# nnanhuang/S3Gaussian

Measured on AMD Instinct MI355X. Metric: train_iters_per_sec, higher is better.
Workload: dtype f32

## Files before the change

### include/s3g_mlp.h

```cpp
#ifndef S3G_MLP_H
#define S3G_MLP_H
#include <stddef.h>
#ifdef __cplusplus
extern "C" {
#endif

typedef struct s3g_mlp_params {
  float *W0, *b0;
  float *P1, *pb1;
  float *P2, *pb2;
  float *S1, *sb1;
  float *S2, *sb2;
  float *D0, *db0;
  float *D1, *db1;
  float *D2, *db2;
} s3g_mlp_params;

size_t s3g_deform_mlp_stash_bytes(int P);
size_t s3g_deform_mlp_pack_bytes(void);

int s3g_deform_mlp_forward(const s3g_mlp_params* w, int P, const float* features, float* dx, float* dshs, float* feat,
                           float* stash, int save_activations, void* stream);

int s3g_deform_mlp_backward(const s3g_mlp_params* w, int P, const float* features, const float* stash, const float* g_dx,
                            const float* g_dshs, const float* g_feat, float* g_features, const s3g_mlp_params* gw,
                            float* workspace, void* stream);

size_t s3g_deform_mlp_wgrad_partial_bytes(void);
int s3g_deform_mlp_backward_ordered(const s3g_mlp_params* w, int P, const float* features, const float* stash, const float* g_dx,
                                    const float* g_dshs, const float* g_feat, float* g_features, const s3g_mlp_params* gw,
                                    float* workspace, float* wgrad_partials, void* stream);

enum { S3G_MLP_F32 = 0, S3G_MLP_BF16X3 = 1, S3G_MLP_BF16X3_ONTHEFLY = 2 };
int s3g_deform_mlp_set_arithmetic(int mode);
int s3g_deform_mlp_get_arithmetic(void);

#include "s3g_hexplane.h"
size_t s3g_deform_infer_workspace_bytes(const s3g_hexplane_desc* d);
int s3g_deform_infer(const s3g_hexplane_desc* d, const s3g_mlp_params* w, int P, const float* xyz, const float* time,
                     const unsigned int* proc_order, float* dx, float* dshs, void* workspace, void* stream);
int s3g_deform_infer_split(const s3g_hexplane_desc* d, const s3g_mlp_params* w, int P, const float* xyz, const float* time,
                           const unsigned int* proc_order, float* dx, float* dshs, void* workspace, void* stream);

#ifdef __cplusplus
}
#endif
#endif
```

### s3gaussian_amd/_lib.py

```python
from __future__ import annotations

import ctypes as C
import os
import subprocess

_HERE = os.path.dirname(os.path.abspath(__file__))
LIB_PATH = os.environ.get("S3G_LIB_PATH") or os.path.join(_HERE, "lib", "libs3g.so")
CSRC_DIR = os.path.join(_HERE, "csrc")

ABI_VERSION = 15

RESIZE_FN = C.CFUNCTYPE(C.c_void_p, C.c_void_p, C.c_size_t)


class RasterInputs(C.Structure):
    _fields_ = [
        ("P", C.c_int), ("D", C.c_int), ("M", C.c_int), ("width", C.c_int), ("height", C.c_int),
        ("background", C.c_void_p), ("means3D", C.c_void_p), ("shs", C.c_void_p), ("colors_precomp", C.c_void_p),
        ("opacities", C.c_void_p), ("scales", C.c_void_p), ("scale_modifier", C.c_float), ("rotations", C.c_void_p),
        ("cov3D_precomp", C.c_void_p), ("viewmatrix", C.c_void_p), ("projmatrix", C.c_void_p), ("cam_pos", C.c_void_p),
        ("tan_fovx", C.c_float), ("tan_fovy", C.c_float), ("prefiltered", C.c_int), ("debug", C.c_int),
    ]


class DensifyAccum(C.Structure):
# ... 106 lines not shown
    if _torch is None:
        _torch, _raw_stream, _cur_device = _bind_fast_paths()
    if _cur_device is not None and getattr(dev, "index", None) is not None and _cur_device() == dev.index:
        return _NULL
    return _torch.cuda.device(dev)


def check(code: int) -> None:
    if code != 0:
        msg = lib().s3g_last_error().decode("utf-8", "replace")
        if code == 1:
            raise Exception(msg)
        raise RuntimeError(f"libs3g error {code}: {msg}")


EXPORTED_SYMBOLS = ["s3g_raster_forward", "s3g_raster_forward_reuse", "s3g_raster_forward_decompose", "s3g_raster_forward2", "s3g_raster_forward_async", "s3g_raster_arena_bytes", "s3g_adam_step_guarded", "s3g_raster_backward", "s3g_raster_backward_workspace_bytes", "s3g_raster_backward2", "s3g_raster_backward2_workspace_bytes", "s3g_hexplane_forward_workspace_bytes", "s3g_knn_workspace_bytes", "s3g_knn_mean_dist2", "s3g_hexplane_forward", "s3g_hexplane_backward", "s3g_hexplane_backward_algo", "s3g_hexplane_backward_workspace_bytes", "s3g_hexplane_backward_scratch_rows", "s3g_hexplane_debug_walk_mask", "s3g_hexplane_set_deterministic", "s3g_hexplane_get_deterministic", "s3g_hexplane_sort_state_words", "s3g_profile_enable", "s3g_profile_read", "s3g_ssim_forward", "s3g_ssim_backward", "s3g_plane_regulation", "s3g_scale_unless_one", "s3g_pixel_losses_forward", "s3g_pixel_losses_combine", "s3g_pixel_losses_backward", "s3g_glue_forward", "s3g_glue_backward", "s3g_deform_mlp_forward", "s3g_deform_mlp_backward", "s3g_deform_mlp_backward_ordered", "s3g_deform_mlp_wgrad_partial_bytes", "s3g_deform_mlp_stash_bytes", "s3g_deform_mlp_pack_bytes", "s3g_deform_mlp_set_arithmetic", "s3g_deform_mlp_get_arithmetic", "s3g_deform_infer", "s3g_deform_infer_split", "s3g_deform_infer_workspace_bytes", "s3g_adam_step", "s3g_densify_stats", "s3g_densify_stats_guarded", "s3g_density_count_words", "s3g_density_classify_densify", "s3g_density_classify_prune", "s3g_density_scan", "s3g_density_apply", "s3g_density_reset_opacity", "s3g_image_metrics_workspace_bytes", "s3g_image_metrics", "s3g_scene_flow_workspace_bytes", "s3g_scene_flow_colors", "s3g_raster_backward_accum", "s3g_raster_backward2_accum", "s3g_mark_visible", "s3g_raster_set_exact_cull", "s3g_raster_get_exact_cull", "s3g_raster_set_bin_band", "s3g_raster_set_backward_wave_bounds", "s3g_last_error", "s3g_abi_version"]
```

### s3gaussian_amd/csrc/mlp.hip

```cpp
#include "mlp_dev.hpp"

namespace s3g {

__global__ void __launch_bounds__(256) mlp_pack_kernel(const s3g_mlp_params w, float* __restrict__ packed) {
  const int k = blockIdx.x, tid = threadIdx.x;
  float* dst = packed + (size_t)k * SLAB;
  if (k == NSLAB) {
    float* bl = packed + (size_t)NSLAB * SLAB;
    const float* src[8] = {w.b0, w.pb1, w.sb1, w.pb2, w.sb2, w.db0, w.db1, w.db2};
    const int n[8] = {64, 64, 64, 3, 48, 64, 64, 3};
    for (int e = tid; e < 8 * 64; e += 256) bl[e] = (e & 63) < n[e >> 6] ? src[e >> 6][e & 63] : 0.f;
    return;
  }
  const float* W = k <= 1 ? w.W0 : k == 2 ? w.P1 : k == 3 ? w.S1 : k == 4 ? w.P2 : k == 5 ? w.S2 : k == 6 ? w.D0 : k == 7 ? w.D1 : w.D2;
  const int out = (k == 4 || k == 8) ? 3 : (k == 5 ? 48 : 64), outpad = (k == 4 || k == 8) ? 32 : 64;
  const int in = k <= 1 ? FEAT : HID, in0 = k == 1 ? 64 : 0, ld = outpad + 1;
  for (int e = tid; e < SLAB; e += 256) dst[e] = 0.f;
  __syncthreads();
  for (int e = tid; e < outpad * 64; e += 256) {
    const int o = e / 64, i = e % 64;
    dst[i * ld + o] = o < out ? W[(size_t)o * in + in0 + i] : 0.f;
  }
}
void mlp_pack_launch(const s3g_mlp_params& w, float* packed, hipStream_t stream) {
// ... 96 lines not shown
      head3_fw(WSLAB(8), BIAS(7), acc, o3, ln);
      store3(o3, a.feat, p0, npts, ln);
    }
    }
    __builtin_amdgcn_sched_barrier(0);
    cur = nxt;
  }
}

struct MlpBwdArgs {
  int P;
  const float* packed;
  const uint32_t* maskbits;
  const float *g_dx, *g_dshs, *g_feat;
  float *g_x, *ws;
};

struct BwdIn {
  float gd[3], gf[3];
  float4 gs[6];
  uint32_t bits[5];
};

template <bool SPLIT>
__global__ void __launch_bounds__(NWAVE * 64) mlp_backward_kernel(const MlpBwdArgs a) {
  extern __shared__ __attribute__((aligned(16))) float lds[];
  const int lane = threadIdx.x & 63, wave = threadIdx.x >> 6;
  load_weights(lds, a.packed, wave, lane);
  const int ntiles = (a.P + MT - 1) / MT;
  const size_t PS = (size_t)a.P * HID;
// ... 20 lines not shown
  };
  const int stride = gridDim.x * NWAVE, t0 = blockIdx.x * NWAVE + wave;
  BwdIn cur, nxt;
  if (t0 < ntiles) issue(cur, t0);
  for (int tile = t0; tile < ntiles; tile += stride) {
    issue(nxt, min(tile + stride, ntiles - 1));
    __builtin_amdgcn_sched_barrier(0);
    const int p0 = tile * MT, npts = min(MT, a.P - p0);
    f32x16 ghid[2], g[2], acc[2], g3[1];
    acc_zero<2>(ghid);
    if (dino) {
      head3(g3, cur.gf);
      acc_zero<2>(acc);
      gemm_reg_t<2, 1, 3>(WSLAB(8), 33, g3, acc, lane);
      masked_bits<2, false>(g, acc, cur.bits[4]);
      act_store<HID, 2, false>(g, a.ws + 0 * PS, 0, p0, npts, lane);
      acc_zero<2>(acc);
      gemm_bw<SPLIT, 2, 2>(WSLAB(7), 65, g, acc, lane);
      masked_bits<2, false>(g, acc, cur.bits[3]);
      act_store<HID, 2, false>(g, a.ws + 1 * PS, 0, p0, npts, lane);
      gemm_bw<SPLIT, 2, 2>(WSLAB(6), 65, g, ghid, lane);
    }
    head3(g3, cur.gd);
    acc_zero<2>(acc);
    gemm_reg_t<2, 1, 3>(WSLAB(4), 33, g3, acc, lane);
    masked_bits<2, false>(g, acc, cur.bits[1]);
    act_store<HID, 2, false>(g, a.ws + 2 * PS, 0, p0, npts, lane);
    acc_zero<2>(acc);
    gemm_bw<SPLIT, 2, 2>(WSLAB(2), 65, g, acc, lane);
    {
      f32x16 gs[2], t[2];
#pragma unroll
      for (int c = 0; c < 8; c++) {
        const float4 v = c < 6 ? cur.gs[c < 6 ? c : 0] : make_float4(0.f, 0.f, 0.f, 0.f);
        gs[c >> 2][4 * (c & 3) + 0] = v.x; gs[c >> 2][4 * (c & 3) + 1] = v.y;
        gs[c >> 2][4 * (c & 3) + 2] = v.z; gs[c >> 2][4 * (c & 3) + 3] = v.w;
      }
      acc_zero<2>(t);
      gemm_bw<SPLIT, 2, 2>(WSLAB(5), 65, gs, t, lane);
      masked_bits<2, false>(g, t, cur.bits[2]);
    }
    act_store<HID, 2, false>(g, a.ws + 3 * PS, 0, p0, npts, lane);
// ... 156 lines not shown
  if (t0 < ntiles) issue(cur, t0);
  for (int tile = t0; tile < ntiles; tile += stride) {
    issue(nxt, min(tile + stride, ntiles - 1));
    __builtin_amdgcn_sched_barrier(0);
    const int p0 = tile * MT, npts = min(MT, a.P - p0);
    int ln = lane;
    asm volatile("" : "+v"(ln));
    f32x16 ghid[2], g[2], acc[2], g3[1];
    ActSplit<2> gsp;
    acc_zero<2>(ghid);
    if (dino) {
      head3(g3, cur.gf);
      acc_zero<2>(acc);
      gemm_reg_t<2, 1, 3>(lds + tbw::D2T, tbw::H3LD, g3, acc, ln);
      masked_bits<2, false>(g, acc, cur.bits[4]);
      act_store<HID, 2, false>(g, a.ws + 0 * PS, 0, p0, npts, ln);
      acc_zero<2>(acc);
      act_split<2, false>(gsp, g);
      gemm_split<2, 2>(wsplit + tbw::D1T, 4, 0, gsp, acc, ln);
      masked_bits<2, false>(g, acc, cur.bits[3]);
      act_store<HID, 2, false>(g, a.ws + 1 * PS, 0, p0, npts, ln);
      act_split<2, false>(gsp, g);
      gemm_split<2, 2>(wsplit + tbw::D0T, 4, 0, gsp, ghid, ln);
    }
    head3(g3, cur.gd);
    acc_zero<2>(acc);
    gemm_reg_t<2, 1, 3>(lds + tbw::P2T, tbw::H3LD, g3, acc, ln);
    masked_bits<2, false>(g, acc, cur.bits[1]);
    act_store<HID, 2, false>(g, a.ws + 2 * PS, 0, p0, npts, ln);
    acc_zero<2>(acc);
    act_split<2, false>(gsp, g);
#pragma unroll
    for (int ks = 0; ks < 4; ks++)
#pragma unroll
      for (int mbo = 0; mbo < 2; mbo++) {
        const float* wr = lds + tbw::P1T + (32 * mbo + (ln & 31)) * tbw::P1LD + 4 * (ln >> 5) + 16 * ks;
        const float4 lo = *reinterpret_cast<const float4*>(wr);
        const float4 hi = *reinterpret_cast<const float4*>(wr + 8);
        const float v[8] = {lo.x, lo.y, lo.z, lo.w, hi.x, hi.y, hi.z, hi.w};
        acc[mbo] = mfma_split(acc[mbo], split8(v), gsp.b[ks >> 1][ks & 1]);
      }
    {
      f32x16 gs[2], t[2];
#pragma unroll
// ... 164 lines not shown
extern "C" size_t s3g_deform_mlp_stash_bytes(int P) {
  return ((size_t)PACK_TOTAL + (size_t)5 * (size_t)(P > 0 ? P : 0) * HID + mask_words(P)) * sizeof(float);
}
extern "C" size_t s3g_deform_mlp_pack_bytes(void) { return (size_t)PACK_TOTAL * sizeof(float); }

static std::atomic<int> g_mlp_arithmetic{S3G_MLP_F32};
extern "C" int s3g_deform_mlp_set_arithmetic(int mode) {
  if (mode != S3G_MLP_F32 && mode != S3G_MLP_BF16X3 && mode != S3G_MLP_BF16X3_ONTHEFLY) {
    set_error("s3g_deform_mlp_set_arithmetic: mode must be S3G_MLP_F32, S3G_MLP_BF16X3 or S3G_MLP_BF16X3_ONTHEFLY");
    return S3G_ERR_INVALID_ARG;
  }
  g_mlp_arithmetic.store(mode, std::memory_order_relaxed);
  return S3G_OK;
}
extern "C" int s3g_deform_mlp_get_arithmetic(void) { return g_mlp_arithmetic.load(std::memory_order_relaxed); }

static int mlp_set_attrs() {
  static std::atomic<uint64_t> done{0};
  if (device_needs_setup(done)) {
    S3G_HIP_CHECK(hipFuncSetAttribute((const void*)mlp_forward_kernel<false>, hipFuncAttributeMaxDynamicSharedMemorySize, MLP_LDS_FLOATS * 4));
    S3G_HIP_CHECK(hipFuncSetAttribute((const void*)mlp_backward_kernel<false>, hipFuncAttributeMaxDynamicSharedMemorySize, MLP_LDS_FLOATS * 4));
    S3G_HIP_CHECK(hipFuncSetAttribute((const void*)mlp_forward_kernel<true>, hipFuncAttributeMaxDynamicSharedMemorySize, MLP_LDS_FLOATS * 4));
    S3G_HIP_CHECK(hipFuncSetAttribute((const void*)mlp_backward_kernel<true>, hipFuncAttributeMaxDynamicSharedMemorySize, MLP_LDS_FLOATS * 4));
    S3G_HIP_CHECK(hipFuncSetAttribute((const void*)mlp_forward_presplit_kernel, hipFuncAttributeMaxDynamicSharedMemorySize, tpw::WORDS * 4));
    S3G_HIP_CHECK(hipFuncSetAttribute((const void*)mlp_backward_presplit_kernel, hipFuncAttributeMaxDynamicSharedMemorySize, tbw::WORDS * 4));
    device_setup_done(done);
  }
  return S3G_OK;
}

// ... 33 lines not shown
}

static int mlp_backward_impl(const s3g_mlp_params* w, int P, const float* features, const float* stash_, const float* g_dx,
                             const float* g_dshs, const float* g_feat, float* g_features, const s3g_mlp_params* gw, float* workspace,
                             float* partials, void* stream_) {
  if (!w || !gw || P < 0 || (P > 0 && (!features || !stash_ || !g_dx || !g_dshs || !g_features || !workspace))) {
    set_error("s3g_deform_mlp_backward: bad argument");
    return S3G_ERR_INVALID_ARG;
  }
  if (P == 0) return S3G_OK;
  if (int e = mlp_set_attrs()) return e;
  hipStream_t stream = (hipStream_t)stream_;
  const float* stash = stash_ + PACK_TOTAL;
  MlpBwdArgs b;
  b.P = P; b.packed = stash_; b.maskbits = reinterpret_cast<const uint32_t*>(stash + (size_t)5 * P * HID); b.g_dx = g_dx; b.g_dshs = g_dshs; b.g_feat = g_feat; b.g_x = g_features; b.ws = workspace;
  const int ntiles = (P + MT - 1) / MT;
  const int blocks = min((ntiles + NWAVE - 1) / NWAVE, 256);
  const int arith = g_mlp_arithmetic.load(std::memory_order_relaxed);
  float* img = const_cast<float*>(stash_) + PACK_FLOATS + tpw::WORDS;
  if (arith == S3G_MLP_BF16X3)
    hipLaunchKernelGGL(mlp_pack_presplit_bwd_kernel, dim3((tbw::WORDS + 255) / 256), dim3(256), 0, stream, *w, reinterpret_cast<uint32_t*>(img));
  else
    mlp_pack_launch(*w, const_cast<float*>(stash_), stream);
  profile_begin(S3G_PROFILE_MLP_BACKWARD, stream);
  if (arith == S3G_MLP_BF16X3) {
    MlpBwdArgs sb = b;
    sb.packed = img;
    hipLaunchKernelGGL(mlp_backward_presplit_kernel, dim3(blocks), dim3(NWAVE * 64), tbw::WORDS * 4, stream, sb);
  } else if (arith != S3G_MLP_F32)
    hipLaunchKernelGGL(mlp_backward_kernel<true>, dim3(blocks), dim3(NWAVE * 64), MLP_LDS_FLOATS * 4, stream, b);
  else
    hipLaunchKernelGGL(mlp_backward_kernel<false>, dim3(blocks), dim3(NWAVE * 64), MLP_LDS_FLOATS * 4, stream, b);
  profile_end(S3G_PROFILE_MLP_BACKWARD, stream, (double)P, 0.0);
  S3G_HIP_CHECK(hipGetLastError());
  profile_begin(S3G_PROFILE_MLP_WGRAD, stream);
  if (int e = mlp_wgrad_launch(P, features, stash, workspace, g_dx, g_dshs, g_feat, gw, partials, stream)) return e;
  profile_end(S3G_PROFILE_MLP_WGRAD, stream, (double)P, 0.0);
  return S3G_OK;
}

extern "C" int s3g_deform_mlp_backward(const s3g_mlp_params* w, int P, const float* features, const float* stash_,
                                       const float* g_dx, const float* g_dshs, const float* g_feat, float* g_features,
                                       const s3g_mlp_params* gw, float* workspace, void* stream_) {
  return mlp_backward_impl(w, P, features, stash_, g_dx, g_dshs, g_feat, g_features, gw, workspace, nullptr, stream_);
}

extern "C" int s3g_deform_mlp_backward_ordered(const s3g_mlp_params* w, int P, const float* features, const float* stash_,
                                               const float* g_dx, const float* g_dshs, const float* g_feat, float* g_features,
                                               const s3g_mlp_params* gw, float* workspace, float* wgrad_partials, void* stream_) {
  if (!wgrad_partials && P > 0) {
    set_error("s3g_deform_mlp_backward_ordered: wgrad_partials is NULL");
// ... 5 lines not shown
```

### s3gaussian_amd/csrc/mlp_dev.hpp

```cpp
#pragma once
#include "common.hpp"

#include "../../include/s3g_mlp.h"

namespace s3g {

typedef float f32x16 __attribute__((ext_vector_type(16)));

constexpr int MT = 32;
constexpr int HID = 64;
constexpr int FEAT = 128;

__device__ __forceinline__ constexpr int rrow(int r) { return (r & 3) + 8 * (r >> 2); }
__device__ __forceinline__ int acc_row(int reg, int lane) { return rrow(reg) + 4 * (lane >> 5); }

template <int MBO, int MBI, bool RELU_IN, int RSTEPS = 16>
__device__ __forceinline__ void gemm_reg(const float* wl, int ld, const f32x16 (&in)[MBI], f32x16 (&acc)[MBO], int lane) {
  const float* base = wl + 4 * (lane >> 5) * ld + (lane & 31);
#pragma unroll
  for (int mbi = 0; mbi < MBI; mbi++)
#pragma unroll
    for (int r = 0; r < RSTEPS; r++) {
      float b = in[mbi][r];
      if (RELU_IN) b = fmaxf(b, 0.f);
// ... 268 lines not shown
constexpr int NSLAB = 9;
constexpr int PACK_FLOATS = NSLAB * SLAB + 8 * 64;
constexpr int NWAVE = 8;
constexpr int MLP_LDS_FLOATS = PACK_FLOATS;

__device__ __forceinline__ void load_weights(float* lds, const float* __restrict__ packed, int wave, int lane) {
  static_assert(PACK_FLOATS % 256 == 0, "image is a whole number of 1 KiB DMA rows");
  for (int c = wave; c < PACK_FLOATS / 256; c += NWAVE)
    __builtin_amdgcn_global_load_lds((const __attribute__((address_space(1))) void*)(packed + c * 256 + lane * 4),
                                     (__attribute__((address_space(3))) void*)(lds + c * 256), 16, 0, 0);
  asm volatile("s_waitcnt vmcnt(0)" ::: "memory");
  __syncthreads();
}

void mlp_pack_launch(const s3g_mlp_params& w, float* packed, hipStream_t stream);
int mlp_wgrad_launch(int P, const float* features, const float* stash, const float* signals, const float* g_dx, const float* g_dshs,
                     const float* g_feat, const s3g_mlp_params* gw, float* partials, hipStream_t stream);

}
```

### s3gaussian_amd/csrc/mlp_wgrad.hip

```cpp
#include "mlp_dev.hpp"

namespace s3g {

constexpr int WG_WAVES = 8;
constexpr int WM_RED = 32 * 2 * 64 + 32 * 2;

struct WJobX {
  const float* G;
  const float* A;
  float* dW;
  float* db;
  int gstride, gw, astride;
  float relu_lo;
  int kind;
  const float* G2;
  const float* A2;
  float* dW2;
  float* db2;
};
struct WAllArgs {
  WJobX job[8];
  int P;
  float* part;
};
constexpr int WPART = 64 * 64 + 64, WPART_BIAS = 64 * 64, WPART_HEAD2 = WPART / 2, WPART_HEAD_BIAS = 3 * 64;
constexpr int WPART_MAX_BLOCKS = 256, WPART_MAX_JOBS = 8;

__device__ __forceinline__ void wgrad_wide_wave(const WJobX& jb, float* __restrict__ red, int P, int lane, float* __restrict__ part) {
  constexpr int STEPS = MT / 2;
  const int i = lane & 31, k = lane >> 5;
  const int gcol = min(2 * i, jb.gw - 2);
  f32x16 acc[2][2];
#pragma unroll
  for (int m = 0; m < 2; m++)
#pragma unroll
    for (int n = 0; n < 2; n++)
#pragma unroll
      for (int r = 0; r < 16; r++) acc[m][n][r] = 0.f;
  float bsum[2] = {0.f, 0.f};
  const int nfull = P / MT, stride = gridDim.x;
  struct Set {
    float g[STEPS][2];
    float v[STEPS][2];
  };
  auto issue = [&](Set& S, int tile) {
    const int p0 = tile * MT;
#pragma unroll
    for (int s = 0; s < STEPS; s++) {
      const float2 x = *reinterpret_cast<const float2*>(jb.G + (size_t)(p0 + 2 * s + k) * jb.gstride + gcol);
      S.g[s][0] = x.x; S.g[s][1] = x.y;
      const float2 y = *reinterpret_cast<const float2*>(jb.A + (size_t)(p0 + 2 * s + k) * jb.astride + 2 * i);
      S.v[s][0] = y.x; S.v[s][1] = y.y;
    }
  };
  auto consume = [&](const Set& S) {
#pragma unroll
    for (int s = 0; s < STEPS; s++) {
      const float b0 = fmaxf(S.v[s][0], jb.relu_lo), b1 = fmaxf(S.v[s][1], jb.relu_lo);
#pragma unroll
      for (int m = 0; m < 2; m++) {
        bsum[m] += S.g[s][m];
        acc[m][0] = __builtin_amdgcn_mfma_f32_32x32x2f32(S.g[s][m], b0, acc[m][0], 0, 0, 0);
        acc[m][1] = __builtin_amdgcn_mfma_f32_32x32x2f32(S.g[s][m], b1, acc[m][1], 0, 0, 0);
      }
    }
  };
  {
    Set A, B;
    const int t0 = blockIdx.x;
    const int cnt = t0 < nfull ? (nfull - t0 + stride - 1) / stride : 0;
    const int last = nfull - 1;
    if (cnt > 0) {
      issue(A, t0);
      for (int it = 0; it < cnt; it += 2) {
        issue(B, min(t0 + (it + 1) * stride, last));
        __builtin_amdgcn_sched_barrier(0);
        consume(A);
        __builtin_amdgcn_sched_barrier(0);
        if (it + 1 >= cnt) break;
        issue(A, min(t0 + (it + 2) * stride, last));
        __builtin_amdgcn_sched_barrier(0);
        consume(B);
        __builtin_amdgcn_sched_barrier(0);
      }
    }
  }
  if (P % MT != 0 && (nfull % stride) == (int)blockIdx.x) {
    const int p0 = nfull * MT;
#pragma unroll
    for (int s = 0; s < STEPS; s++) {
      const int p = p0 + 2 * s + k;
      float ga[2] = {0.f, 0.f}, ba[2] = {0.f, 0.f};
      if (p < P) {
        ga[0] = jb.G[(size_t)p * jb.gstride + gcol]; ga[1] = jb.G[(size_t)p * jb.gstride + gcol + 1];
        ba[0] = fmaxf(jb.A[(size_t)p * jb.astride + 2 * i], jb.relu_lo);
        ba[1] = fmaxf(jb.A[(size_t)p * jb.astride + 2 * i + 1], jb.relu_lo);
      }
#pragma unroll
      for (int m = 0; m < 2; m++) {
        bsum[m] += ga[m];
#pragma unroll
        for (int n = 0; n < 2; n++) acc[m][n] = __builtin_amdgcn_mfma_f32_32x32x2f32(ga[m], ba[n], acc[m][n], 0, 0, 0);
      }
    }
  }
#pragma unroll
  for (int m = 0; m < 2; m++)
#pragma unroll
    for (int n = 0; n < 2; n++)
// ... 98 lines not shown
    for (int e = lane; e < 3 * 64; e += 64) part[e] = red[e];
    if (lane < 3) part[WPART_HEAD_BIAS + lane] = red[3 * 64 + lane];
  } else {
    for (int e = lane; e < 3 * 64; e += 64) atomicAdd(&dW[e], red[e]);
    if (db != nullptr && lane < 3) atomicAdd(&db[lane], red[3 * 64 + lane]);
  }
  wave_lds_sync();
}

__global__ void __launch_bounds__(WG_WAVES * 64) mlp_wgrad_all_kernel(const WAllArgs a) {
  extern __shared__ __attribute__((aligned(16))) float red_all[];
  const int lane = threadIdx.x & 63, wave = __builtin_amdgcn_readfirstlane(threadIdx.x >> 6);
  const WJobX jb = a.job[wave];
  float* red = red_all + wave * WM_RED;
  float* part = a.part ? a.part + ((size_t)blockIdx.x * (blockDim.x >> 6) + wave) * WPART : nullptr;
  if (jb.kind == 0) {
    wgrad_wide_wave(jb, red, a.P, lane, part);
  } else {
    wgrad_head_wave(jb.G, jb.A, jb.dW, jb.db, red, a.P, lane, part);
    if (jb.G2 != nullptr) wgrad_head_wave(jb.G2, jb.A2, jb.dW2, jb.db2, red, a.P, lane, part ? part + WPART_HEAD2 : nullptr);
  }
}

__global__ void __launch_bounds__(256) mlp_wgrad_reduce_kernel(const WAllArgs a, int nb, int njobs) {
  __shared__ float quarter[4][64];
  const int j = blockIdx.y, lane = threadIdx.x & 63, wv = threadIdx.x >> 6;
  const int e = blockIdx.x * 64 + lane;
  const WJobX jb = a.job[j];
  float* dst = nullptr;
  if (jb.kind == 0) {
    if (e < jb.gw * 64) dst = jb.dW + (size_t)(e >> 6) * jb.astride + (e & 63);
    else if (e >= WPART_BIAS && e < WPART_BIAS + jb.gw && jb.db != nullptr) dst = jb.db + (e - WPART_BIAS);
  } else {
    const int h = e >= WPART_HEAD2 ? 1 : 0, r = e - h * WPART_HEAD2;
    float* dW = h ? jb.dW2 : jb.dW;
    float* db = h ? jb.db2 : jb.db;
    if (h == 0 || jb.G2 != nullptr) {
      if (r < 3 * 64) dst = dW + r;
      else if (r >= WPART_HEAD_BIAS && r < WPART_HEAD_BIAS + 3 && db != nullptr) dst = db + (r - WPART_HEAD_BIAS);
    }
  }
  float s = 0.f;
  if (dst != nullptr && e < WPART) {
    const size_t stride = (size_t)njobs * WPART;
    const int per = (nb + 3) / 4, b0 = wv * per, b1 = min(nb, b0 + per);
// ... 16 lines not shown
static int launch_wgrad_all(const WJobX* jobs, int njobs, int P, hipStream_t stream, float* partials) {
  WAllArgs a;
  memset(&a, 0, sizeof a);
  for (int j = 0; j < njobs; j++) a.job[j] = jobs[j];
  a.P = P;
  a.part = partials;
  const int ntiles = (P + MT - 1) / MT;
  const int blocks = min(ntiles, WPART_MAX_BLOCKS);
  hipLaunchKernelGGL(mlp_wgrad_all_kernel, dim3(blocks), dim3(njobs * 64), (size_t)njobs * WM_RED * sizeof(float), stream, a);
  if (partials != nullptr)
    hipLaunchKernelGGL(mlp_wgrad_reduce_kernel, dim3((WPART + 63) / 64, njobs), dim3(256), 0, stream, a, blocks, njobs);
  S3G_HIP_CHECK(hipGetLastError());
  return S3G_OK;
}

int mlp_wgrad_launch(int P, const float* features, const float* stash, const float* signals, const float* g_dx, const float* g_dshs,
                     const float* g_feat, const s3g_mlp_params* gw, float* partials, hipStream_t stream) {
  static std::atomic<uint64_t> done{0};
  if (device_needs_setup(done)) {
    S3G_HIP_CHECK(hipFuncSetAttribute((const void*)mlp_wgrad_all_kernel, hipFuncAttributeMaxDynamicSharedMemorySize, WPART_MAX_JOBS * WM_RED * 4));
    device_setup_done(done);
  }
  const size_t PS = (size_t)P * HID;
  const float NONE = -__builtin_huge_valf(), RELU = 0.f;
  auto wide = [](const float* G, const float* A, float* dW, float* db, int astride, float relu_lo, int gw = HID) {
    return WJobX{G, A, dW, db, gw, gw, astride, relu_lo, 0, nullptr, nullptr, nullptr, nullptr};
  };
  const WJobX w0a = wide(signals + 4 * PS, features, gw->W0, gw->b0, FEAT, NONE);
  const WJobX w0b = wide(signals + 4 * PS, features + 64, gw->W0 + 64, nullptr, FEAT, NONE);
  const WJobX d0 = wide(signals + 1 * PS, stash + 0 * PS, gw->D0, gw->db0, HID, NONE);
  const WJobX d1 = wide(signals + 0 * PS, stash + 3 * PS, gw->D1, gw->db1, HID, NONE);
  const WJobX p1 = wide(signals + 2 * PS, stash + 0 * PS, gw->P1, gw->pb1, HID, RELU);
  const WJobX s1 = wide(signals + 3 * PS, stash + 0 * PS, gw->S1, gw->sb1, HID, RELU);
  const WJobX s2 = wide(g_dshs, stash + 2 * PS, gw->S2, gw->sb2, HID, NONE, 48);
  WJobX head{g_dx, stash + 1 * PS, gw->P2, gw->pb2, 3, 3, HID, NONE, 1, nullptr, nullptr, nullptr, nullptr};
  if (g_feat != nullptr) {
    head.G2 = g_feat; head.A2 = stash + 4 * PS; head.dW2 = gw->D2; head.db2 = gw->db2;
    const WJobX jobs[8] = {w0a, w0b, d0, p1, s1, d1, s2, head};
    return launch_wgrad_all(jobs, 8, P, stream, partials);
  }
  const WJobX jobs[6] = {w0a, w0b, p1, s1, s2, head};
  return launch_wgrad_all(jobs, 6, P, stream, partials);
}

}

extern "C" size_t s3g_deform_mlp_wgrad_partial_bytes(void) {
  return (size_t)s3g::WPART_MAX_BLOCKS * s3g::WPART_MAX_JOBS * s3g::WPART * sizeof(float);
}
```

### s3gaussian_amd/csrc/raster_forward.hip

```cpp
#include "geom_math.hpp"

#include <stdarg.h>

#include <vector>

namespace s3g {

static thread_local char g_err[512] = {0};
void set_error(const char* fmt, ...) {
  va_list ap;
  va_start(ap, fmt);
  vsnprintf(g_err, sizeof g_err, fmt, ap);
  va_end(ap);
}

static bool g_exact_cull = true;
static int g_max_tiles_lds = MAX_TILES_LDS;

struct ProfRec { hipEvent_t a, b; double instances, pixels; };
static bool g_prof_on = false;
static std::vector<ProfRec> g_prof[S3G_PROFILE_IDS];
static hipEvent_t g_prof_pending[S3G_PROFILE_IDS];
void profile_begin(int id, hipStream_t stream) {
  if (!g_prof_on || id < 0 || id >= S3G_PROFILE_IDS) return;
// ... 813 lines not shown
                                                            const float* __restrict__ viewmatrix,
                                                            uint8_t* __restrict__ present) {
  const int idx = blockIdx.x * 256 + threadIdx.x;
  if (idx >= P) return;
  const float3 p = make_float3(means3D[3 * idx], means3D[3 * idx + 1], means3D[3 * idx + 2]);
  present[idx] = xform_4x3(p, viewmatrix).z > 0.2f ? 1 : 0;
}

static inline uint32_t round_up8(uint32_t v) { return (v + 7u) & ~7u; }

}

using namespace s3g;

extern "C" const char* s3g_last_error(void) { return g_err; }
extern "C" int s3g_abi_version(void) { return 15; }

static int raster_forward_impl(const s3g_raster_inputs* in, const float* colors2, float* out_color2,
                               s3g_resize_fn geometry_buffer, void* geometry_user, s3g_resize_fn binning_buffer,
                               void* binning_user, s3g_resize_fn image_buffer, void* image_user, float* out_color,
                               float* out_depth, int* radii, int* num_rendered, void* stream_,
                               const s3g_raster_async* as = nullptr) {
  g_err[0] = 0;
  hipStream_t stream = (hipStream_t)stream_;
  if (!in || (!as && (!geometry_buffer || !binning_buffer || !image_buffer || !num_rendered))) {
    set_error("s3g_raster_forward: NULL argument");
    return S3G_ERR_INVALID_ARG;
  }
  if (as && (!as->geometry_arena || !as->image_arena || !as->binning_arena || as->capacity_instances == 0 ||
             as->capacity_instances > 0x7fffffffu || as->capacity_slots < as->capacity_instances)) {
    set_error("s3g_raster_forward_async: needs the three arenas and 0 < capacity_instances <= capacity_slots");
// ... 319 lines not shown
```

### s3gaussian_amd/mlp.py

```python
from __future__ import annotations

import ctypes as C
import os

import torch

from . import _lib

_NAMES = ["W0", "b0", "P1", "pb1", "P2", "pb2", "S1", "sb1", "S2", "sb2", "D0", "db0", "D1", "db1", "D2", "db2"]
_SHAPES = [(64, 128), (64,), (64, 64), (64,), (3, 64), (3,), (64, 64), (64,), (48, 64), (48,), (64, 64), (64,), (64, 64),
           (64,), (3, 64), (3,)]


class _Params(C.Structure):
    _fields_ = [(n, C.c_void_p) for n in _NAMES]


_bound = False


def _bind():
    global _bound
    L = _lib.lib()
    if not _bound:
# ... 6 lines not shown
        L.s3g_deform_mlp_backward.restype = C.c_int
        L.s3g_deform_mlp_backward.argtypes = [C.POINTER(_Params), C.c_int, vp, vp, vp, vp, vp, vp, C.POINTER(_Params), vp, vp]
        L.s3g_deform_mlp_backward_ordered.restype = C.c_int
        L.s3g_deform_mlp_backward_ordered.argtypes = [C.POINTER(_Params), C.c_int, vp, vp, vp, vp, vp, vp, C.POINTER(_Params), vp, vp, vp]
        L.s3g_deform_mlp_wgrad_partial_bytes.restype = C.c_size_t
        from .hexplane import _HexDesc
        L.s3g_deform_infer_workspace_bytes.restype = C.c_size_t
        L.s3g_deform_infer_workspace_bytes.argtypes = [C.POINTER(_HexDesc)]
        L.s3g_deform_infer.restype = C.c_int
        L.s3g_deform_infer.argtypes = [C.POINTER(_HexDesc), C.POINTER(_Params), C.c_int, vp, vp, vp, vp, vp, vp, vp]
        L.s3g_deform_infer_split.restype = C.c_int
        L.s3g_deform_infer_split.argtypes = L.s3g_deform_infer.argtypes
        L.s3g_deform_mlp_set_arithmetic.restype = C.c_int
        L.s3g_deform_mlp_set_arithmetic.argtypes = [C.c_int]
        L.s3g_deform_mlp_get_arithmetic.restype = C.c_int
        _bound = True
        set_mlp_arithmetic(os.environ.get("S3G_MLP_ARITHMETIC") or DEFAULT_ARITHMETIC)
    return L


_ARITHMETIC = {"f32": 0, "bf16x3": 1, "bf16x3_onthefly": 2}
DEFAULT_ARITHMETIC = "bf16x3"
ORDERED_WGRAD_FLUSH = os.environ.get("S3G_MLP_ORDERED_WGRAD", "1") != "0"


def set_mlp_arithmetic(mode: str) -> None:
    if mode not in _ARITHMETIC:
        raise ValueError(f"set_mlp_arithmetic: mode must be one of {sorted(_ARITHMETIC)}, got {mode!r}")
    _lib.check(_bind().s3g_deform_mlp_set_arithmetic(_ARITHMETIC[mode]))


def get_mlp_arithmetic() -> str:
    v = _bind().s3g_deform_mlp_get_arithmetic()
    return next(k for k, x in _ARITHMETIC.items() if x == v)


def _pack(tensors) -> _Params:
    p = _Params()
    for n, shape, t in zip(_NAMES, _SHAPES, tensors):
        if tuple(t.shape) != shape or t.dtype != torch.float32 or not t.is_contiguous():
            raise RuntimeError(f"deform MLP: parameter {n} must be contiguous float32 {shape}, got {tuple(t.shape)} {t.dtype}")
        setattr(p, n, t.data_ptr())
    return p


class _DeformMLP(torch.autograd.Function):
    @staticmethod
    def forward(ctx, features, need_feat, grad_mode, *params):
        if not features.is_cuda:
# ... 22 lines not shown
        x, stash, *params = ctx.saved_tensors
        L = _bind()
        P, dev = x.shape[0], x.device
        z = lambda g, n: (torch.zeros((P, n), dtype=torch.float32, device=dev) if g is None else g.contiguous().float())
        g_dx, g_dshs = z(g_dx, 3), z(g_dshs, 48)
        no_feat = g_feat is None
        g_feat = None if no_feat else g_feat.contiguous().float()
        gx = torch.empty_like(x)
        flat = torch.zeros(sum(p.numel() for p in params), dtype=torch.float32, device=dev)
        grads, off = [], 0
        for p in params:
            grads.append(flat[off:off + p.numel()].view(p.shape))
            off += p.numel()
        ws = torch.empty((5, P, 64), dtype=torch.float32, device=dev)
        w, gw = _pack([p.detach() for p in params]), _pack(grads)
        with _lib.on_device(dev):
            if ORDERED_WGRAD_FLUSH:
                part = torch.empty(L.s3g_deform_mlp_wgrad_partial_bytes() // 4, dtype=torch.float32, device=dev)
                _lib.check(L.s3g_deform_mlp_backward_ordered(C.byref(w), P, x.data_ptr(), stash.data_ptr(), g_dx.data_ptr(),
                                                             g_dshs.data_ptr(), None if no_feat else g_feat.data_ptr(), gx.data_ptr(),
                                                             C.byref(gw), ws.data_ptr(), part.data_ptr(), _lib.stream_ptr()))
            else:
                _lib.check(L.s3g_deform_mlp_backward(C.byref(w), P, x.data_ptr(), stash.data_ptr(), g_dx.data_ptr(),
                                                     g_dshs.data_ptr(), None if no_feat else g_feat.data_ptr(), gx.data_ptr(),
                                                     C.byref(gw), ws.data_ptr(), _lib.stream_ptr()))
        if no_feat:
            grads = [None if n.startswith(("D", "db")) else g for n, g in zip(_NAMES, grads)]
        return (gx, None, None, *grads)


def _head_params(feature_out, pos_deform, shs_deform, dino_head):
    return [feature_out[0].weight, feature_out[0].bias, pos_deform[1].weight, pos_deform[1].bias, pos_deform[3].weight,
            pos_deform[3].bias, shs_deform[1].weight, shs_deform[1].bias, shs_deform[3].weight, shs_deform[3].bias,
            dino_head[0].weight, dino_head[0].bias, dino_head[2].weight, dino_head[2].bias, dino_head[4].weight,
            dino_head[4].bias]


@torch.no_grad()
def deform_infer(grid, xyz, time, feature_out, pos_deform, shs_deform, dino_head, uniform_time=None, arithmetic="f32"):
    if arithmetic not in ("f32", "bf16x3"):
# ... 31 lines not shown
```

Before: 144.0.

## Rebuild head-layer gradient signals in wgrad instead of storing them

The backward kernel no longer writes the P1 and D1 pre-activation gradient signals (two P x 64 float buffers) to the workspace by default. The weight-gradient kernel instead recomputes them from the 3-wide head gradients, the head weights and the stashed mask bits, using cross-lane permutes. This trades global memory writes and reads for extra ALU work and permutes inside the wgrad job. It also adds a mode switch exposed through a new ABI entry point.

```diff
diff --git a/include/s3g_mlp.h b/include/s3g_mlp.h
--- a/include/s3g_mlp.h
+++ b/include/s3g_mlp.h
@@ -35,6 +35,10 @@
 int s3g_deform_mlp_set_arithmetic(int mode);
 int s3g_deform_mlp_get_arithmetic(void);
 
+enum { S3G_MLP_HEAD_SIGNALS_REBUILT = 0, S3G_MLP_HEAD_SIGNALS_STORED = 1 };
+int s3g_deform_mlp_set_head_signals(int mode);
+int s3g_deform_mlp_get_head_signals(void);
+
 #include "s3g_hexplane.h"
 size_t s3g_deform_infer_workspace_bytes(const s3g_hexplane_desc* d);
 int s3g_deform_infer(const s3g_hexplane_desc* d, const s3g_mlp_params* w, int P, const float* xyz, const float* time,
diff --git a/s3gaussian_amd/_lib.py b/s3gaussian_amd/_lib.py
--- a/s3gaussian_amd/_lib.py
+++ b/s3gaussian_amd/_lib.py
@@ -8,7 +8,7 @@
 LIB_PATH = os.environ.get("S3G_LIB_PATH") or os.path.join(_HERE, "lib", "libs3g.so")
 CSRC_DIR = os.path.join(_HERE, "csrc")
 
-ABI_VERSION = 15
+ABI_VERSION = 16
 
 RESIZE_FN = C.CFUNCTYPE(C.c_void_p, C.c_void_p, C.c_size_t)
 
@@ -145,4 +145,4 @@
         raise RuntimeError(f"libs3g error {code}: {msg}")
 
 
-EXPORTED_SYMBOLS = ["s3g_raster_forward", "s3g_raster_forward_reuse", "s3g_raster_forward_decompose", "s3g_raster_forward2", "s3g_raster_forward_async", "s3g_raster_arena_bytes", "s3g_adam_step_guarded", "s3g_raster_backward", "s3g_raster_backward_workspace_bytes", "s3g_raster_backward2", "s3g_raster_backward2_workspace_bytes", "s3g_hexplane_forward_workspace_bytes", "s3g_knn_workspace_bytes", "s3g_knn_mean_dist2", "s3g_hexplane_forward", "s3g_hexplane_backward", "s3g_hexplane_backward_algo", "s3g_hexplane_backward_workspace_bytes", "s3g_hexplane_backward_scratch_rows", "s3g_hexplane_debug_walk_mask", "s3g_hexplane_set_deterministic", "s3g_hexplane_get_deterministic", "s3g_hexplane_sort_state_words", "s3g_profile_enable", "s3g_profile_read", "s3g_ssim_forward", "s3g_ssim_backward", "s3g_plane_regulation", "s3g_scale_unless_one", "s3g_pixel_losses_forward", "s3g_pixel_losses_combine", "s3g_pixel_losses_backward", "s3g_glue_forward", "s3g_glue_backward", "s3g_deform_mlp_forward", "s3g_deform_mlp_backward", "s3g_deform_mlp_backward_ordered", "s3g_deform_mlp_wgrad_partial_bytes", "s3g_deform_mlp_stash_bytes", "s3g_deform_mlp_pack_bytes", "s3g_deform_mlp_set_arithmetic", "s3g_deform_mlp_get_arithmetic", "s3g_deform_infer", "s3g_deform_infer_split", "s3g_deform_infer_workspace_bytes", "s3g_adam_step", "s3g_densify_stats", "s3g_densify_stats_guarded", "s3g_density_count_words", "s3g_density_classify_densify", "s3g_density_classify_prune", "s3g_density_scan", "s3g_density_apply", "s3g_density_reset_opacity", "s3g_image_metrics_workspace_bytes", "s3g_image_metrics", "s3g_scene_flow_workspace_bytes", "s3g_scene_flow_colors", "s3g_raster_backward_accum", "s3g_raster_backward2_accum", "s3g_mark_visible", "s3g_raster_set_exact_cull", "s3g_raster_get_exact_cull", "s3g_raster_set_bin_band", "s3g_raster_set_backward_wave_bounds", "s3g_last_error", "s3g_abi_version"]
+EXPORTED_SYMBOLS = ["s3g_raster_forward", "s3g_raster_forward_reuse", "s3g_raster_forward_decompose", "s3g_raster_forward2", "s3g_raster_forward_async", "s3g_raster_arena_bytes", "s3g_adam_step_guarded", "s3g_raster_backward", "s3g_raster_backward_workspace_bytes", "s3g_raster_backward2", "s3g_raster_backward2_workspace_bytes", "s3g_hexplane_forward_workspace_bytes", "s3g_knn_workspace_bytes", "s3g_knn_mean_dist2", "s3g_hexplane_forward", "s3g_hexplane_backward", "s3g_hexplane_backward_algo", "s3g_hexplane_backward_workspace_bytes", "s3g_hexplane_backward_scratch_rows", "s3g_hexplane_debug_walk_mask", "s3g_hexplane_set_deterministic", "s3g_hexplane_get_deterministic", "s3g_hexplane_sort_state_words", "s3g_profile_enable", "s3g_profile_read", "s3g_ssim_forward", "s3g_ssim_backward", "s3g_plane_regulation", "s3g_scale_unless_one", "s3g_pixel_losses_forward", "s3g_pixel_losses_combine", "s3g_pixel_losses_backward", "s3g_glue_forward", "s3g_glue_backward", "s3g_deform_mlp_forward", "s3g_deform_mlp_backward", "s3g_deform_mlp_backward_ordered", "s3g_deform_mlp_wgrad_partial_bytes", "s3g_deform_mlp_stash_bytes", "s3g_deform_mlp_pack_bytes", "s3g_deform_mlp_set_arithmetic", "s3g_deform_mlp_get_arithmetic", "s3g_deform_mlp_set_head_signals", "s3g_deform_mlp_get_head_signals", "s3g_deform_infer", "s3g_deform_infer_split", "s3g_deform_infer_workspace_bytes", "s3g_adam_step", "s3g_densify_stats", "s3g_densify_stats_guarded", "s3g_density_count_words", "s3g_density_classify_densify", "s3g_density_classify_prune", "s3g_density_scan", "s3g_density_apply", "s3g_density_reset_opacity", "s3g_image_metrics_workspace_bytes", "s3g_image_metrics", "s3g_scene_flow_workspace_bytes", "s3g_scene_flow_colors", "s3g_raster_backward_accum", "s3g_raster_backward2_accum", "s3g_mark_visible", "s3g_raster_set_exact_cull", "s3g_raster_get_exact_cull", "s3g_raster_set_bin_band", "s3g_raster_set_backward_wave_bounds", "s3g_last_error", "s3g_abi_version"]
diff --git a/s3gaussian_amd/csrc/mlp.hip b/s3gaussian_amd/csrc/mlp.hip
--- a/s3gaussian_amd/csrc/mlp.hip
+++ b/s3gaussian_amd/csrc/mlp.hip
@@ -134,6 +134,7 @@
   const uint32_t* maskbits;
   const float *g_dx, *g_dshs, *g_feat;
   float *g_x, *ws;
+  int store_heads;
 };
 
 struct BwdIn {
@@ -184,7 +185,7 @@
       acc_zero<2>(acc);
       gemm_reg_t<2, 1, 3>(WSLAB(8), 33, g3, acc, lane);
       masked_bits<2, false>(g, acc, cur.bits[4]);
-      act_store<HID, 2, false>(g, a.ws + 0 * PS, 0, p0, npts, lane);
+      if (a.store_heads) act_store<HID, 2, false>(g, a.ws + 0 * PS, 0, p0, npts, lane);
       acc_zero<2>(acc);
       gemm_bw<SPLIT, 2, 2>(WSLAB(7), 65, g, acc, lane);
       masked_bits<2, false>(g, acc, cur.bits[3]);
@@ -195,7 +196,7 @@
     acc_zero<2>(acc);
     gemm_reg_t<2, 1, 3>(WSLAB(4), 33, g3, acc, lane);
     masked_bits<2, false>(g, acc, cur.bits[1]);
-    act_store<HID, 2, false>(g, a.ws + 2 * PS, 0, p0, npts, lane);
+    if (a.store_heads) act_store<HID, 2, false>(g, a.ws + 2 * PS, 0, p0, npts, lane);
     acc_zero<2>(acc);
     gemm_bw<SPLIT, 2, 2>(WSLAB(2), 65, g, acc, lane);
     {
@@ -382,7 +383,7 @@
       acc_zero<2>(acc);
       gemm_reg_t<2, 1, 3>(lds + tbw::D2T, tbw::H3LD, g3, acc, ln);
       masked_bits<2, false>(g, acc, cur.bits[4]);
-      act_store<HID, 2, false>(g, a.ws + 0 * PS, 0, p0, npts, ln);
+      if (a.store_heads) act_store<HID, 2, false>(g, a.ws + 0 * PS, 0, p0, npts, ln);
       acc_zero<2>(acc);
       act_split<2, false>(gsp, g);
       gemm_split<2, 2>(wsplit + tbw::D1T, 4, 0, gsp, acc, ln);
@@ -395,7 +396,7 @@
     acc_zero<2>(acc);
     gemm_reg_t<2, 1, 3>(lds + tbw::P2T, tbw::H3LD, g3, acc, ln);
     masked_bits<2, false>(g, acc, cur.bits[1]);
-    act_store<HID, 2, false>(g, a.ws + 2 * PS, 0, p0, npts, ln);
+    if (a.store_heads) act_store<HID, 2, false>(g, a.ws + 2 * PS, 0, p0, npts, ln);
     acc_zero<2>(acc);
     act_split<2, false>(gsp, g);
 #pragma unroll
@@ -590,6 +591,17 @@
   return S3G_OK;
 }
 extern "C" int s3g_deform_mlp_get_arithmetic(void) { return g_mlp_arithmetic.load(std::memory_order_relaxed); }
+
+static std::atomic<int> g_mlp_head_signals{S3G_MLP_HEAD_SIGNALS_STORED};
+extern "C" int s3g_deform_mlp_set_head_signals(int mode) {
+  if (mode != S3G_MLP_HEAD_SIGNALS_REBUILT && mode != S3G_MLP_HEAD_SIGNALS_STORED) {
+    set_error("s3g_deform_mlp_set_head_signals: mode must be S3G_MLP_HEAD_SIGNALS_REBUILT or S3G_MLP_HEAD_SIGNALS_STORED");
+    return S3G_ERR_INVALID_ARG;
+  }
+  g_mlp_head_signals.store(mode, std::memory_order_relaxed);
+  return S3G_OK;
+}
+extern "C" int s3g_deform_mlp_get_head_signals(void) { return g_mlp_head_signals.load(std::memory_order_relaxed); }
 
 static int mlp_set_attrs() {
   static std::atomic<uint64_t> done{0};
@@ -653,6 +665,8 @@
   const float* stash = stash_ + PACK_TOTAL;
   MlpBwdArgs b;
   b.P = P; b.packed = stash_; b.maskbits = reinterpret_cast<const uint32_t*>(stash + (size_t)5 * P * HID); b.g_dx = g_dx; b.g_dshs = g_dshs; b.g_feat = g_feat; b.g_x = g_features; b.ws = workspace;
+  const bool rebuild_heads = g_mlp_head_signals.load(std::memory_order_relaxed) == S3G_MLP_HEAD_SIGNALS_REBUILT;
+  b.store_heads = rebuild_heads ? 0 : 1;
   const int ntiles = (P + MT - 1) / MT;
   const int blocks = min((ntiles + NWAVE - 1) / NWAVE, 256);
   const int arith = g_mlp_arithmetic.load(std::memory_order_relaxed);
@@ -673,7 +687,7 @@
   profile_end(S3G_PROFILE_MLP_BACKWARD, stream, (double)P, 0.0);
   S3G_HIP_CHECK(hipGetLastError());
   profile_begin(S3G_PROFILE_MLP_WGRAD, stream);
-  if (int e = mlp_wgrad_launch(P, features, stash, workspace, g_dx, g_dshs, g_feat, gw, partials, stream)) return e;
+  if (int e = mlp_wgrad_launch(P, features, stash, b.maskbits, workspace, g_dx, g_dshs, g_feat, w, gw, rebuild_heads, partials, stream)) return e;
   profile_end(S3G_PROFILE_MLP_WGRAD, stream, (double)P, 0.0);
   return S3G_OK;
 }
diff --git a/s3gaussian_amd/csrc/mlp_dev.hpp b/s3gaussian_amd/csrc/mlp_dev.hpp
--- a/s3gaussian_amd/csrc/mlp_dev.hpp
+++ b/s3gaussian_amd/csrc/mlp_dev.hpp
@@ -306,7 +306,8 @@
 }
 
 void mlp_pack_launch(const s3g_mlp_params& w, float* packed, hipStream_t stream);
-int mlp_wgrad_launch(int P, const float* features, const float* stash, const float* signals, const float* g_dx, const float* g_dshs,
-                     const float* g_feat, const s3g_mlp_params* gw, float* partials, hipStream_t stream);
-
-}
+int mlp_wgrad_launch(int P, const float* features, const float* stash, const uint32_t* maskbits, const float* signals, const float* g_dx,
+                     const float* g_dshs, const float* g_feat, const s3g_mlp_params* w, const s3g_mlp_params* gw, bool rebuild_heads,
+                     float* partials, hipStream_t stream);
+
+}
diff --git a/s3gaussian_amd/csrc/mlp_wgrad.hip b/s3gaussian_amd/csrc/mlp_wgrad.hip
--- a/s3gaussian_amd/csrc/mlp_wgrad.hip
+++ b/s3gaussian_amd/csrc/mlp_wgrad.hip
@@ -17,6 +17,9 @@
   const float* A2;
   float* dW2;
   float* db2;
+  const uint32_t* bits;
+  const float* Wh;
+  const float* g3;
 };
 struct WAllArgs {
   WJobX job[8];
@@ -29,7 +32,25 @@
 __device__ __forceinline__ void wgrad_wide_wave(const WJobX& jb, float* __restrict__ red, int P, int lane, float* __restrict__ part) {
   constexpr int STEPS = MT / 2;
   const int i = lane & 31, k = lane >> 5;
-  const int gcol = min(2 * i, jb.gw - 2);
+  const bool rebuilt = jb.kind == 2;
+  const int gcol = rebuilt ? k : min(2 * i, jb.gw - 2);
+  const int hsel = (i >> 1) & 1, bit0 = 16 * (i >> 4) + 2 * (i & 1) + 4 * ((i & 15) >> 2);
+  const int pick = 4 * (k + 32 * hsel);
+  float wh[3][2] = {{0.f, 0.f}, {0.f, 0.f}, {0.f, 0.f}};
+  if (rebuilt) {
+#pragma unroll
+    for (int c = 0; c < 3; c++) {
+      const float2 x = *reinterpret_cast<const float2*>(jb.Wh + c * HID + 2 * i);
+      wh[c][0] = x.x; wh[c][1] = x.y;
+    }
+  }
+  auto rebuild = [&](float x0, float x1, float x2, uint32_t word, float (&ga)[2]) {
+#pragma unroll
+    for (int m = 0; m < 2; m++) {
+      const float v = __builtin_fmaf(wh[2][m], x2, __builtin_fmaf(wh[1][m], x1, wh[0][m] * x0));
+      ga[m] = ((word >> (bit0 + m)) & 1u) ? v : 0.f;
+    }
+  };
   f32x16 acc[2][2];
 #pragma unroll
   for (int m = 0; m < 2; m++)
@@ -42,9 +63,14 @@
   struct Set {
     float g[STEPS][2];
     float v[STEPS][2];
+    uint32_t word;
+    float third;
   };
   auto issue = [&](Set& S, int tile) {
     const int p0 = tile * MT;
+    const int rt = rebuilt ? tile : 0;
+    S.word = jb.bits[(size_t)rt * 5 * 64 + lane];
+    S.third = jb.g3[(size_t)(rt * MT + i) * 3 + ((lane & 1) ? 0 : 2)];
 #pragma unroll
     for (int s = 0; s < STEPS; s++) {
       const float2 x = *reinterpret_cast<const float2*>(jb.G + (size_t)(p0 + 2 * s + k) * jb.gstride + gcol);
@@ -57,11 +83,17 @@
 #pragma unroll
     for (int s = 0; s < STEPS; s++) {
       const float b0 = fmaxf(S.v[s][0], jb.relu_lo), b1 = fmaxf(S.v[s][1], jb.relu_lo);
+      float ga[2] = {S.g[s][0], S.g[s][1]};
+      if (rebuilt) {
+        const uint32_t word = (uint32_t)__builtin_amdgcn_ds_bpermute(pick + 8 * s, (int)S.word);
+        const float c = __int_as_float(__builtin_amdgcn_ds_bpermute(pick + 8 * s, __float_as_int(S.third)));
+        rebuild(k ? c : ga[0], k ? ga[0] : ga[1], k ? ga[1] : c, word, ga);
+      }
 #pragma unroll
       for (int m = 0; m < 2; m++) {
-        bsum[m] += S.g[s][m];
-        acc[m][0] = __builtin_amdgcn_mfma_f32_32x32x2f32(S.g[s][m], b0, acc[m][0], 0, 0, 0);
-        acc[m][1] = __builtin_amdgcn_mfma_f32_32x32x2f32(S.g[s][m], b1, acc[m][1], 0, 0, 0);
+        bsum[m] += ga[m];
+        acc[m][0] = __builtin_amdgcn_mfma_f32_32x32x2f32(ga[m], b0, acc[m][0], 0, 0, 0);
+        acc[m][1] = __builtin_amdgcn_mfma_f32_32x32x2f32(ga[m], b1, acc[m][1], 0, 0, 0);
       }
     }
   };
@@ -92,7 +124,12 @@
       const int p = p0 + 2 * s + k;
       float ga[2] = {0.f, 0.f}, ba[2] = {0.f, 0.f};
       if (p < P) {
-        ga[0] = jb.G[(size_t)p * jb.gstride + gcol]; ga[1] = jb.G[(size_t)p * jb.gstride + gcol + 1];
+        if (rebuilt) {
+          const float* row = jb.G + (size_t)p * 3;
+          rebuild(row[0], row[1], row[2], jb.bits[(size_t)nfull * 5 * 64 + 2 * s + k + 32 * hsel], ga);
+        } else {
+          ga[0] = jb.G[(size_t)p * jb.gstride + gcol]; ga[1] = jb.G[(size_t)p * jb.gstride + gcol + 1];
+        }
         ba[0] = fmaxf(jb.A[(size_t)p * jb.astride + 2 * i], jb.relu_lo);
         ba[1] = fmaxf(jb.A[(size_t)p * jb.astride + 2 * i + 1], jb.relu_lo);
       }
@@ -221,7 +258,7 @@
   const WJobX jb = a.job[wave];
   float* red = red_all + wave * WM_RED;
   float* part = a.part ? a.part + ((size_t)blockIdx.x * (blockDim.x >> 6) + wave) * WPART : nullptr;
-  if (jb.kind == 0) {
+  if (jb.kind != 1) {
     wgrad_wide_wave(jb, red, a.P, lane, part);
   } else {
     wgrad_head_wave(jb.G, jb.A, jb.dW, jb.db, red, a.P, lane, part);
@@ -235,7 +272,7 @@
   const int e = blockIdx.x * 64 + lane;
   const WJobX jb = a.job[j];
   float* dst = nullptr;
-  if (jb.kind == 0) {
+  if (jb.kind != 1) {
     if (e < jb.gw * 64) dst = jb.dW + (size_t)(e >> 6) * jb.astride + (e & 63);
     else if (e >= WPART_BIAS && e < WPART_BIAS + jb.gw && jb.db != nullptr) dst = jb.db + (e - WPART_BIAS);
   } else {
@@ -282,8 +319,9 @@
   return S3G_OK;
 }
 
-int mlp_wgrad_launch(int P, const float* features, const float* stash, const float* signals, const float* g_dx, const float* g_dshs,
-                     const float* g_feat, const s3g_mlp_params* gw, float* partials, hipStream_t stream) {
+int mlp_wgrad_launch(int P, const float* features, const float* stash, const uint32_t* maskbits, const float* signals, const float* g_dx,
+                     const float* g_dshs, const float* g_feat, const s3g_mlp_params* w, const s3g_mlp_params* gw, bool rebuild_heads,
+                     float* partials, hipStream_t stream) {
   static std::atomic<uint64_t> done{0};
   if (device_needs_setup(done)) {
     S3G_HIP_CHECK(hipFuncSetAttribute((const void*)mlp_wgrad_all_kernel, hipFuncAttributeMaxDynamicSharedMemorySize, WPART_MAX_JOBS * WM_RED * 4));
@@ -291,17 +329,22 @@
   }
   const size_t PS = (size_t)P * HID;
   const float NONE = -__builtin_huge_valf(), RELU = 0.f;
-  auto wide = [](const float* G, const float* A, float* dW, float* db, int astride, float relu_lo, int gw = HID) {
-    return WJobX{G, A, dW, db, gw, gw, astride, relu_lo, 0, nullptr, nullptr, nullptr, nullptr};
+  auto wide = [&](const float* G, const float* A, float* dW, float* db, int astride, float relu_lo, int gw = HID) {
+    return WJobX{G, A, dW, db, gw, gw, astride, relu_lo, 0, nullptr, nullptr, nullptr, nullptr, maskbits + 1 * 64, nullptr, g_dx};
+  };
+  auto rebuilt = [&](const float* g, int plane, const float* Wh, const float* A, float* dW, float* db, float relu_lo) {
+    return WJobX{g, A, dW, db, 3, HID, HID, relu_lo, 2, nullptr, nullptr, nullptr, nullptr, maskbits + plane * 64, Wh, g};
   };
   const WJobX w0a = wide(signals + 4 * PS, features, gw->W0, gw->b0, FEAT, NONE);
   const WJobX w0b = wide(signals + 4 * PS, features + 64, gw->W0 + 64, nullptr, FEAT, NONE);
   const WJobX d0 = wide(signals + 1 * PS, stash + 0 * PS, gw->D0, gw->db0, HID, NONE);
-  const WJobX d1 = wide(signals + 0 * PS, stash + 3 * PS, gw->D1, gw->db1, HID, NONE);
-  const WJobX p1 = wide(signals + 2 * PS, stash + 0 * PS, gw->P1, gw->pb1, HID, RELU);
+  const WJobX d1 = rebuild_heads && g_feat != nullptr ? rebuilt(g_feat, 4, w->D2, stash + 3 * PS, gw->D1, gw->db1, NONE)
+                                                      : wide(signals + 0 * PS, stash + 3 * PS, gw->D1, gw->db1, HID, NONE);
+  const WJobX p1 = rebuild_heads ? rebuilt(g_dx, 1, w->P2, stash + 0 * PS, gw->P1, gw->pb1, RELU)
+                                 : wide(signals + 2 * PS, stash + 0 * PS, gw->P1, gw->pb1, HID, RELU);
   const WJobX s1 = wide(signals + 3 * PS, stash + 0 * PS, gw->S1, gw->sb1, HID, RELU);
   const WJobX s2 = wide(g_dshs, stash + 2 * PS, gw->S2, gw->sb2, HID, NONE, 48);
-  WJobX head{g_dx, stash + 1 * PS, gw->P2, gw->pb2, 3, 3, HID, NONE, 1, nullptr, nullptr, nullptr, nullptr};
+  WJobX head{g_dx, stash + 1 * PS, gw->P2, gw->pb2, 3, 3, HID, NONE, 1, nullptr, nullptr, nullptr, nullptr, nullptr, nullptr, nullptr};
   if (g_feat != nullptr) {
     head.G2 = g_feat; head.A2 = stash + 4 * PS; head.dW2 = gw->D2; head.db2 = gw->db2;
     const WJobX jobs[8] = {w0a, w0b, d0, p1, s1, d1, s2, head};
diff --git a/s3gaussian_amd/csrc/raster_forward.hip b/s3gaussian_amd/csrc/raster_forward.hip
--- a/s3gaussian_amd/csrc/raster_forward.hip
+++ b/s3gaussian_amd/csrc/raster_forward.hip
@@ -851,7 +851,7 @@
 using namespace s3g;
 
 extern "C" const char* s3g_last_error(void) { return g_err; }
-extern "C" int s3g_abi_version(void) { return 15; }
+extern "C" int s3g_abi_version(void) { return 16; }
 
 static int raster_forward_impl(const s3g_raster_inputs* in, const float* colors2, float* out_color2,
                                s3g_resize_fn geometry_buffer, void* geometry_user, s3g_resize_fn binning_buffer,
diff --git a/s3gaussian_amd/mlp.py b/s3gaussian_amd/mlp.py
--- a/s3gaussian_amd/mlp.py
+++ b/s3gaussian_amd/mlp.py
@@ -44,8 +44,12 @@
         L.s3g_deform_mlp_set_arithmetic.restype = C.c_int
         L.s3g_deform_mlp_set_arithmetic.argtypes = [C.c_int]
         L.s3g_deform_mlp_get_arithmetic.restype = C.c_int
+        L.s3g_deform_mlp_set_head_signals.restype = C.c_int
+        L.s3g_deform_mlp_set_head_signals.argtypes = [C.c_int]
+        L.s3g_deform_mlp_get_head_signals.restype = C.c_int
         _bound = True
         set_mlp_arithmetic(os.environ.get("S3G_MLP_ARITHMETIC") or DEFAULT_ARITHMETIC)
+        reset_mlp_head_signals()
     return L
 
 
@@ -63,6 +67,34 @@
 def get_mlp_arithmetic() -> str:
     v = _bind().s3g_deform_mlp_get_arithmetic()
     return next(k for k, x in _ARITHMETIC.items() if x == v)
+
+
+_HEAD_SIGNALS = {"rebuilt": 0, "stored": 1}
+DEFAULT_HEAD_SIGNALS = "rebuilt"
+LIBRARY_HEAD_SIGNALS = "stored"
+HEAD_SIGNALS = DEFAULT_HEAD_SIGNALS
+
+
+def set_mlp_head_signals(mode: str) -> None:
+    global HEAD_SIGNALS
+    if mode not in _HEAD_SIGNALS:
+        raise ValueError(f"set_mlp_head_signals: mode must be one of {sorted(_HEAD_SIGNALS)}, got {mode!r}")
+    _lib.check(_bind().s3g_deform_mlp_set_head_signals(_HEAD_SIGNALS[mode]))
+    HEAD_SIGNALS = mode
+
+
+def reset_mlp_head_signals() -> None:
+    global HEAD_SIGNALS
+    mode = os.environ.get("S3G_MLP_HEAD_SIGNALS") or DEFAULT_HEAD_SIGNALS
+    if mode not in _HEAD_SIGNALS:
+        raise ValueError(f"S3G_MLP_HEAD_SIGNALS must be one of {sorted(_HEAD_SIGNALS)}, got {mode!r}")
+    _lib.check(_lib.lib().s3g_deform_mlp_set_head_signals(_HEAD_SIGNALS[LIBRARY_HEAD_SIGNALS]))
+    HEAD_SIGNALS = mode
+
+
+def get_mlp_head_signals() -> str:
+    v = _bind().s3g_deform_mlp_get_head_signals()
+    return next(k for k, x in _HEAD_SIGNALS.items() if x == v)
 
 
 def _pack(tensors) -> _Params:
@@ -115,16 +147,23 @@
             off += p.numel()
         ws = torch.empty((5, P, 64), dtype=torch.float32, device=dev)
         w, gw = _pack([p.detach() for p in params]), _pack(grads)
-        with _lib.on_device(dev):
-            if ORDERED_WGRAD_FLUSH:
-                part = torch.empty(L.s3g_deform_mlp_wgrad_partial_bytes() // 4, dtype=torch.float32, device=dev)
-                _lib.check(L.s3g_deform_mlp_backward_ordered(C.byref(w), P, x.data_ptr(), stash.data_ptr(), g_dx.data_ptr(),
-                                                             g_dshs.data_ptr(), None if no_feat else g_feat.data_ptr(), gx.data_ptr(),
-                                                             C.byref(gw), ws.data_ptr(), part.data_ptr(), _lib.stream_ptr()))
-            else:
-                _lib.check(L.s3g_deform_mlp_backward(C.byref(w), P, x.data_ptr(), stash.data_ptr(), g_dx.data_ptr(),
-                                                     g_dshs.data_ptr(), None if no_feat else g_feat.data_ptr(), gx.data_ptr(),
-                                                     C.byref(gw), ws.data_ptr(), _lib.stream_ptr()))
+        prev, want = L.s3g_deform_mlp_get_head_signals(), _HEAD_SIGNALS[HEAD_SIGNALS]
+        if prev != want:
+            L.s3g_deform_mlp_set_head_signals(want)
+        try:
+            with _lib.on_device(dev):
+                if ORDERED_WGRAD_FLUSH:
+                    part = torch.empty(L.s3g_deform_mlp_wgrad_partial_bytes() // 4, dtype=torch.float32, device=dev)
+                    _lib.check(L.s3g_deform_mlp_backward_ordered(C.byref(w), P, x.data_ptr(), stash.data_ptr(), g_dx.data_ptr(),
+                                                                 g_dshs.data_ptr(), None if no_feat else g_feat.data_ptr(), gx.data_ptr(),
+                                                                 C.byref(gw), ws.data_ptr(), part.data_ptr(), _lib.stream_ptr()))
+                else:
+                    _lib.check(L.s3g_deform_mlp_backward(C.byref(w), P, x.data_ptr(), stash.data_ptr(), g_dx.data_ptr(),
+                                                         g_dshs.data_ptr(), None if no_feat else g_feat.data_ptr(), gx.data_ptr(),
+                                                         C.byref(gw), ws.data_ptr(), _lib.stream_ptr()))
+        finally:
+            if prev != want:
+                L.s3g_deform_mlp_set_head_signals(prev)
         if no_feat:
             grads = [None if n.startswith(("D", "db")) else g for n, g in zip(_NAMES, grads)]
         return (gx, None, None, *grads)
```

Measured after the change: 143.4, median of 3. Within noise of the previous version (-0.4%).
